# xbpeng/DeepMimic

Hardware: NVIDIA H100
Metric: env-steps/sec (30 Hz policy steps; humanoid3d_spinkick, 4096 envs/GPU) (higher is better)
Workload: dtype f32

## Files before the change

deepmimic_b200/csrc/kernels/dm_step.cu:

```cuda
#include "dm_model.cuh"
#include <type_traits>

namespace dmk {

namespace {

template <int W>
struct Tl {
    static __device__ __forceinline__ float shfl(float v, int src) { return __shfl_sync(0xffffffffu, v, src, W); }
    static __device__ __forceinline__ int shfli(int v, int src) { return __shfl_sync(0xffffffffu, v, src, W); }
    static __device__ __forceinline__ V3 shfl3(V3 v, int src) { return mk3(shfl(v.x, src), shfl(v.y, src), shfl(v.z, src)); }
    static __device__ __forceinline__ S6 shfl6(S6 v, int src) { return mks(shfl3(v.a, src), shfl3(v.l, src)); }
};
__device__ __forceinline__ void ld12(const float* p, float* o) {
    const float4 a = reinterpret_cast<const float4*>(p)[0], b = reinterpret_cast<const float4*>(p)[1], c_ = reinterpret_cast<const float4*>(p)[2];
    o[0] = a.x; o[1] = a.y; o[2] = a.z; o[3] = a.w; o[4] = b.x; o[5] = b.y; o[6] = b.z; o[7] = b.w; o[8] = c_.x; o[9] = c_.y; o[10] = c_.z; o[11] = c_.w;
}
__device__ __forceinline__ void st12(float* p, const float* o) {
    reinterpret_cast<float4*>(p)[0] = make_float4(o[0], o[1], o[2], o[3]); reinterpret_cast<float4*>(p)[1] = make_float4(o[4], o[5], o[6], o[7]);
    reinterpret_cast<float4*>(p)[2] = make_float4(o[8], o[9], o[10], o[11]);
}
__device__ __forceinline__ float rcp_fast(float x) { float r; asm("rcp.approx.ftz.f32 %0, %1;" : "=f"(r) : "f"(x)); return r; }
__device__ __forceinline__ int wmax(int v) {
#pragma unroll
    for (int o = 16; o > 0; o >>= 1) v = max(v, __shfl_xor_sync(0xffffffffu, v, o));
    return v;
}

struct Art {
    float ww[6];
    float wv[9];
    float vv[6];
};
__device__ __forceinline__ V3 wvT_mul(const float* g, V3 w) { return mk3(g[0] * w.x + g[3] * w.y + g[6] * w.z, g[1] * w.x + g[4] * w.y + g[7] * w.z, g[2] * w.x + g[5] * w.y + g[8] * w.z); }
__device__ __forceinline__ void rot_sym(const M3& R, const float* s, float* o) {
    float t[9];
#pragma unroll
    for (int j = 0; j < 3; ++j) {
        t[0 + j] = s[0] * R.m[j] + s[1] * R.m[3 + j] + s[2] * R.m[6 + j];
        t[3 + j] = s[1] * R.m[j] + s[3] * R.m[3 + j] + s[4] * R.m[6 + j];
        t[6 + j] = s[2] * R.m[j] + s[4] * R.m[3 + j] + s[5] * R.m[6 + j];
    }
    o[0] = R.m[0] * t[0] + R.m[3] * t[3] + R.m[6] * t[6];
    o[1] = R.m[0] * t[1] + R.m[3] * t[4] + R.m[6] * t[7];
    o[2] = R.m[0] * t[2] + R.m[3] * t[5] + R.m[6] * t[8];
    o[3] = R.m[1] * t[1] + R.m[4] * t[4] + R.m[7] * t[7];
    o[4] = R.m[1] * t[2] + R.m[4] * t[5] + R.m[7] * t[8];
    o[5] = R.m[2] * t[2] + R.m[5] * t[5] + R.m[8] * t[8];
}
__device__ __forceinline__ float normalize_angle3(float t) {
    float n = fmodf(t, 6.283185307179586f);
    if (n > 3.14159265358979f) n -= 6.283185307179586f;
    else if (n < -3.14159265358979f) n += 6.283185307179586f;
    return n;
}
__device__ __forceinline__ V3 quat_rotvec3(Q4 q) {
    float s = sqrtf(q.x * q.x + q.y * q.y + q.z * q.z);
    if (!(s > 0.000001f)) return mk3(0.f, 0.f, 0.f);
    float th = normalize_angle3(2.0f * atan2f(s, q.w));
    float k = th / s;
    return mk3(q.x * k, q.y * k, q.z * k);
}
__device__ __forceinline__ Q4 quat_integrate3(V3 omega, Q4 quat, bool base_body, float dt) {
    V3 angvel = base_body ? omega : qrot(quat, omega);
    float fAngle = sqrtf(dot(angvel, angvel));
    const float kThr = 0.5f * 1.57079632679489661923f;
    if (fAngle * dt > kThr) fAngle = kThr / dt;
    V3 axis;
    if (fAngle < 0.001f) axis = angvel * (0.5f * dt - (dt * dt * dt) * 0.020833333333f * fAngle * fAngle);
    else axis = angvel * (__sinf(0.5f * fAngle * dt) / fAngle);
    float cw = __cosf(fAngle * dt * 0.5f);
    Q4 r = base_body ? qmul(quat, mkq(-axis.x, -axis.y, -axis.z, cw)) : qmul(mkq(axis.x, axis.y, axis.z, cw), quat);
    float n = rsqrtf(r.x * r.x + r.y * r.y + r.z * r.z + r.w * r.w);
    return mkq(r.x * n, r.y * n, r.z * n, r.w * n);
}

enum LkSlot { kLC = 0 , kLM = 3,
              kLD = 4 , kLThr = 7,
              kLWd = 8 , kLInt = 14 , kLInt2 = 15 ,
              kLWb = 16 , kLFlg = 22 , kLTree = 23 ,
              kLAx = 24 , kLTl = 27,
              kLZr = 28 ,
              kLHe = 32 , kLKp = 35,
              kLKd = 36, kLLo = 37, kLHi = 38, kLChild = 39 ,
              kLDc = 40 , kLMc = 43 ,
              kLDyn = 44 , kLDChild = 45 ,
              kLkFloats = 48 };
__device__ __forceinline__ float4 ld4(const float* p) { return *reinterpret_cast<const float4*>(p); }
enum HdrSlot { kHLayout = 0, kHLvc = 24, kHGrav = 32 , kHh = 35, kHScale = 36, kHMu = 37, kHFdt = 38, kHDmax = 39 , kHdrFloats = 40 };
__device__ __forceinline__ float* step_smem() { extern __shared__ __align__(16) float dm_step_sm[]; return dm_step_sm; }

}

int dm_step_layout(int nl, int n, int chain_len, int maxrows, int W, StepLayout* L) {
    const int maxpts = maxrows / 3;
    int o = 0;
    L->nl = nl; L->n = n; L->chain_len = chain_len; L->maxrows = maxrows; L->maxpts = maxpts;
    L->oU = o; o += nl * 24;
    L->oR = o; o += nl * 12;
    L->oA = o;
    const int world = nl * 24, tri = maxrows * (maxrows + 1) / 2;
    L->oW = o; L->oV = o + nl * 12;
    L->oPp = o + world; L->oQ = L->oPp + maxpts * 4;
    const int pre = world + maxpts * 4 + 4 * 8;
    o += (pre > tri ? pre : tri);
    o = (o + 3) & ~3;
    const int ys = dm_step_y_stride(W), scr = 28 * (nl - 1);
    L->oY = o; o += (chain_len * ys > scr) ? chain_len * ys : scr;
    L->oLam = o; o += maxrows; o += (o & 1); L->oRhs = o; o += maxrows; L->oInv = o; o += maxrows;
    L->oRl = o; o += maxrows;
    L->oPi = o; o += maxpts; L->oPr = o; o += maxpts;
    L->oG = o; o += 21 + 13 + 2;
    L->oZ = o; o += ((n + 3) / 4) * 4;
    L->env_floats = ((o + 15) / 32) * 32 + 16;
    L->hot_floats = kHdrFloats + ((nl * kLkFloats + (nl * nl + nl * chain_len + 3) / 4 + 3) / 4) * 4;
    return L->hot_floats * 4 + 0;
}
int dm_step_smem_bytes(const StepLayout& L, int tiles) { return (L.hot_floats + L.env_floats * tiles) * static_cast<int>(sizeof(float)); }

constexpr int kSubstepBarriers = 2;
constexpr int kPgsBlock = 2;
enum PgsSection { kSecLimit = 0, kSecNormal = 1, kSecFriction = 2 };
// ... 808 lines not shown
            x[i] *= sG[15 + i];
        }
        dB = mks(mk3(x[0], x[1], x[2]), mk3(x[3], x[4], x[5]));
#pragma unroll
        for (int i = 0; i < 6; ++i) sB[7 + i] = cl100(sB[7 + i] + x[i]);
    }
    float z0 = 0.f, z1 = 0.f, z2 = 0.f, qd0 = 0.f, qd1 = 0.f, qd2 = 0.f;
    if (c.ndof >= 1) z0 = sZ[dof0] * u[21];
    if (c.ndof == 3) { z1 = sZ[dof0 + 1] * u[22]; z2 = sZ[dof0 + 2] * u[23]; }
    auto descend = [&](S6 a) {
        if (c.ndof >= 1) { qd0 = z0 - u[18] * (a.a.x * u[0] + a.a.y * u[1] + a.a.z * u[2] + a.l.x * u[3] + a.l.y * u[4] + a.l.z * u[5]); a.a += qd0 * S0; }
        if (c.ndof == 3) {
            qd1 = z1 - u[19] * (a.a.x * u[6] + a.a.y * u[7] + a.a.z * u[8] + a.l.x * u[9] + a.l.y * u[10] + a.l.z * u[11]); a.a += qd1 * S1;
            qd2 = z2 - u[20] * (a.a.x * u[12] + a.a.y * u[13] + a.a.z * u[14] + a.l.x * u[15] + a.l.y * u[16] + a.l.z * u[17]); a.a += qd2 * S2;
        }
        return a;
    };
    S6 al = mks(mk3(0, 0, 0), mk3(0, 0, 0));
    if (c.lane == 0) al = dB;
#pragma unroll 1
    for (int lv = 0; lv <= dmax; ++lv) {
        S6 pa = T::shfl6(al, dpar);
        if (dlev == lv) al = descend(shift_m(pa, cw));
    }
    __syncwarp();
    return make_float3(qd0, qd1, qd2);
}

template <int W>
__device__ __noinline__ void vel_pass(float jvx, float jvy, float jvz, bool want) {
    const Ctx c = make_ctx<W>();
    using T = Tl<W>;
    const StepLayout& LY = lay_of(c);
    const float* sS = c.E + LY.oR; float* sV = c.E + LY.oV; const float* sB = c.E + LY.oG + 21;
    float q[12];
    ld12(sS + c.li * 12, q);
    const V3 S0 = mk3(q[0], q[1], q[2]), S1 = mk3(q[3], q[4], q[5]), S2 = mk3(q[6], q[7], q[8]), cw = mk3(q[9], q[10], q[11]);
    V3 jww = mk3(0, 0, 0);
    if (c.jtype == kJSpherical) jww = jvx * S0 + jvy * S1 + jvz * S2; else if (c.jtype == kJRevolute) jww = jvx * S0;
    S6 vel = mks(mk3(0, 0, 0), mk3(0, 0, 0));
    if (c.lane == 0) { const V3 bo = mk3(sB[7], sB[8], sB[9]); vel = mks(bo + jww, mk3(sB[10], sB[11], sB[12]) + cross(bo, cw)); }
#pragma unroll 1
    for (int lv = 1; lv <= c.maxlevel; ++lv) {
        const S6 pv = T::shfl6(vel, c.plane);
        if (c.level == lv) vel = mks(pv.a + jww, pv.l + cross(pv.a, cw));
    }
    if (c.act && want) {
        float* v = sV + c.lane * 12;
        v[0] = vel.a.x; v[1] = vel.a.y; v[2] = vel.a.z; v[3] = vel.l.x; v[4] = vel.l.y; v[5] = vel.l.z;
    }
    __syncwarp();
}

template <int W, bool TASK>
__global__ void __launch_bounds__(kStepMaxThreads, 1) dm_step_kernel(const DevModel* __restrict__ gm, DevState st, const double* __restrict__ frame_times,
                                                                       const float* __restrict__ frames, double dt, int n_updates, int sim_substeps, StepLayout LY) {
    using T = Tl<W>;
    extern __shared__ __align__(16) float sm[];
    const int tiles = blockDim.x / W;
    const int tile = threadIdx.x / W;
    const int lane = threadIdx.x % W;
    const int slot = blockIdx.x * tiles + tile;
    const int env = (W == 16 && st.order) ? st.order[slot] : slot;
    const DevModel& M = *gm;
    const int nl = LY.nl, CL = LY.chain_len;
    const bool act = lane < nl;
    const int li = act ? lane : nl - 1;

    float* LK = sm + kHdrFloats;
    unsigned char* CD = reinterpret_cast<unsigned char*>(LK + nl * kLkFloats);
    unsigned char* CH = CD + nl * nl;
    int* LYS = reinterpret_cast<int*>(sm + kHLayout);
    for (int j = threadIdx.x; j < nl; j += blockDim.x) {
        const DevLink& K = M.link[j];
        float* q = LK + j * kLkFloats;
        const int p = K.parent;
        for (int k = 0; k < 3; ++k) { q[kLC + k] = K.evec[k] + (p >= 0 ? M.link[p].dvec[k] : 0.f); q[kLD + k] = K.dvec[k]; q[kLAx + k] = K.axis[k]; }
        q[kLM] = K.mass;
        auto lumped = [&](int c_) { const DevLink& C_ = M.link[c_]; return C_.ndof == 0 && C_.nchild == 0 && C_.parent >= 0 && M.link[C_.parent].ndof > 0; };
        const bool isroot = p < 0, self_lumped = lumped(j);
        {
            float cm = 0.f, mdx = 0.f, mdy = 0.f, mdz = 0.f, wD[6] = {0, 0, 0, 0, 0, 0}, wB[6] = {0, 0, 0, 0, 0, 0};
            auto add_part = [&](float m_, V3 r, const float* iD, const float* iB) {
                const float rr = dot(r, r);
                const float sh[6] = {m_ * (rr - r.x * r.x), -m_ * r.x * r.y, -m_ * r.x * r.z, m_ * (rr - r.y * r.y), -m_ * r.y * r.z, m_ * (rr - r.z * r.z)};
                for (int k = 0; k < 6; ++k) { wD[k] += iD[k] + sh[k]; wB[k] += iB[k] + sh[k]; }
                cm += m_; mdx += m_ * r.x; mdy += m_ * r.y; mdz += m_ * r.z;
            };
            if (!self_lumped) {
                V3 r = mk3(K.dvec[0], K.dvec[1], K.dvec[2]);
                if (isroot) r = r + mul(qmat(mkq(K.zrot[0], K.zrot[1], K.zrot[2], K.zrot[3])), mk3(K.evec[0], K.evec[1], K.evec[2]));
                const float iD[6] = {K.inertiaD[0], 0.f, 0.f, K.inertiaD[1], 0.f, K.inertiaD[2]}, iB[6] = {K.inertiaB[0], 0.f, 0.f, K.inertiaB[1], 0.f, K.inertiaB[2]};
                add_part(K.mass, r, iD, iB);
                for (int k = 0; k < K.nchild; ++k) {
                    const int c_ = K.child[k];
                    if (!lumped(c_)) continue;
                    const DevLink& C_ = M.link[c_];
                    const M3 Rc = qmat(mkq(C_.zrot[0], C_.zrot[1], C_.zrot[2], C_.zrot[3]));
                    const V3 rc = mk3(C_.evec[0] + K.dvec[0], C_.evec[1] + K.dvec[1], C_.evec[2] + K.dvec[2]) + mulT(Rc, mk3(C_.dvec[0], C_.dvec[1], C_.dvec[2]));
                    const float cD[6] = {C_.inertiaD[0], 0.f, 0.f, C_.inertiaD[1], 0.f, C_.inertiaD[2]}, cB[6] = {C_.inertiaB[0], 0.f, 0.f, C_.inertiaB[1], 0.f, C_.inertiaB[2]};
                    float rD[6], rB[6];
                    rot_sym(Rc, cD, rD); rot_sym(Rc, cB, rB);
                    add_part(C_.mass, rc, rD, rB);
                }
            }
            for (int k = 0; k < 6; ++k) { q[kLWd + k] = wD[k]; q[kLWb + k] = wB[k]; }
            q[kLMc] = cm;
            const float icm = cm > 0.f ? 1.0f / cm : 0.f;
            q[kLDc] = mdx * icm; q[kLDc + 1] = mdy * icm; q[kLDc + 2] = mdz * icm;
            int dch = 0, dn = 0;
            for (int k = 0; k < K.nchild; ++k) if (!lumped(K.child[k])) { dch |= (K.child[k] & 0xff) << (8 * dn); ++dn; }
            const int dlev = isroot ? -1 : (self_lumped ? 100 : K.level - 1);
            const int dpar = isroot ? 0 : p, byp = (!isroot && p >= 0 && M.link[p].parent < 0) ? p : 0xff;
            reinterpret_cast<int*>(q)[kLDyn] = (dpar & 0xff) | ((dlev & 0xff) << 8) | ((byp & 0xff) << 16) | ((dn & 0xff) << 24);
            reinterpret_cast<int*>(q)[kLDChild] = dch;
        }
        reinterpret_cast<int*>(q)[kLInt] = (K.parent & 0xff) | ((K.jtype & 0xff) << 8) | ((K.ndof & 0xff) << 16) | ((K.depth0 & 0xff) << 24);
        reinterpret_cast<int*>(q)[kLInt2] = (K.dof0 & 0xff) | ((K.last_depth & 0xff) << 8) | ((K.nchild & 0xff) << 16);
        for (int k = 0; k < 4; ++k) q[kLZr + k] = K.zrot[k];
        for (int k = 0; k < 3; ++k) q[kLHe + k] = K.he[k];
        q[kLThr] = K.break_thr; q[kLKp] = K.kp; q[kLKd] = K.kd; q[kLTl] = K.tlim; q[kLLo] = K.lim_lo; q[kLHi] = K.lim_hi;
        reinterpret_cast<int*>(q)[kLFlg] = (K.shape & 0xff) | ((K.fall_contact & 0xff) << 8) | ((K.has_limit & 0xff) << 16);
        reinterpret_cast<int*>(q)[kLTree] = (K.level & 0xff) | ((M.maxlevel & 0xff) << 8) | ((K.nchild & 0xff) << 16);
        reinterpret_cast<int*>(q)[kLChild] = (K.child[0] & 0xff) | ((K.child[1] & 0xff) << 8) | ((K.child[2] & 0xff) << 16) | ((K.child[3] & 0xff) << 24);
        for (int d = 0; d < CL; ++d) CH[j * CL + d] = M.chain_dof[j][d];
        for (int b = 0; b < nl; ++b) {
            int cnt = 0;
            const int lim = min(K.last_depth, M.link[b].last_depth);
            while (cnt <= lim && M.chain_dof[j][cnt] == M.chain_dof[b][cnt]) ++cnt;
            CD[j * nl + b] = static_cast<unsigned char>(cnt);
        }
    }
    if (threadIdx.x == blockDim.x - 1) {
        static_assert(sizeof(StepLayout) / sizeof(int) <= kHLvc, "StepLayout must fit the header slot");
        const int* src = reinterpret_cast<const int*>(&LY);
        for (int k = 0; k < static_cast<int>(sizeof(StepLayout) / sizeof(int)); ++k) LYS[k] = src[k];
        sm[kHGrav] = M.gravity[0]; sm[kHGrav + 1] = M.gravity[1]; sm[kHGrav + 2] = M.gravity[2];
        sm[kHh] = static_cast<float>(dt) / static_cast<float>(sim_substeps); sm[kHScale] = M.scale; sm[kHMu] = M.friction; sm[kHFdt] = static_cast<float>(dt);
    }
    if (threadIdx.x == 8) {
        int mx = 0;
        for (int j = 0; j < nl; ++j) { const DevLink& K = M.link[j]; if (K.parent >= 0 && !(K.ndof == 0 && K.nchild == 0 && M.link[K.parent].ndof > 0)) mx = max(mx, K.level - 1); }
        reinterpret_cast<int*>(sm)[kHDmax] = mx;
    }
    __syncthreads();

    float* E = sm + LY.hot_floats + tile * LY.env_floats;
    for (int k = lane * 4; k < LY.env_floats; k += W * 4) *reinterpret_cast<float4*>(E + k) = make_float4(0.f, 0.f, 0.f, 0.f);
    __syncwarp();
    float* sV = E + LY.oV; float* sG = E + LY.oG; float* sQ = E + LY.oQ; float* sLam = E + LY.oLam;
    const float* LKo = LK + li * kLkFloats;
    const int jtype = (reinterpret_cast<const int*>(LKo)[kLInt] >> 8) & 0xff, ndof = act ? ((reinterpret_cast<const int*>(LKo)[kLInt] >> 16) & 0xff) : 0;
    const int lflags = reinterpret_cast<const int*>(LKo)[kLFlg];
    const bool fall_contact = ((lflags >> 8) & 0xff) != 0, has_limit = ((lflags >> 16) & 0xff) != 0;

    const int ss = sim_stride(nl);
    float* sim = st.sim + static_cast<size_t>(env) * ss;
    double* tm = st.time + static_cast<size_t>(env) * kTimeDoubles;
    int* fl = st.flags + static_cast<size_t>(env) * kFlagInts;
    float* mani = st.manifold + static_cast<size_t>(env) * nl * kManifoldFloats;
    double* tk = nullptr;
    double* tkx = nullptr;
    if constexpr (TASK) { tk = st.task + static_cast<size_t>(env) * kTaskDoubles; tkx = st.taskx + static_cast<size_t>(env) * kTaskExtDoubles; }
    float* sB = sG + 21;
    if (lane == 0) {
        float4 b0 = reinterpret_cast<const float4*>(sim)[0], b1 = reinterpret_cast<const float4*>(sim)[1], b2 = reinterpret_cast<const float4*>(sim)[2],
               b3 = reinterpret_cast<const float4*>(sim)[3];
        sB[0] = b0.x; sB[1] = b0.y; sB[2] = b0.z; sB[3] = b1.x; sB[4] = b1.y; sB[5] = b1.z; sB[6] = b1.w;
        sB[7] = b2.x; sB[8] = b2.y; sB[9] = b2.z; sB[10] = b3.x; sB[11] = b3.y; sB[12] = b3.z;
    }
    float4 jp = reinterpret_cast<const float4*>(sim + 16)[li];
    float4 jv = reinterpret_cast<const float4*>(sim + 16 + 4 * nl)[li];
    int need_action = fl[kFNeedAction];
    int cbits = 0;
    bool alive = fl[kFDone] == 0;
    int f_over = fl[kFRowOverflow], f_updates = fl[kFUpdates];
    __syncwarp();

    const float h = static_cast<float>(dt) / static_cast<float>(sim_substeps);
    const float fdt = static_cast<float>(dt);
    const float gx = M.gravity[0], gy = M.gravity[1], gz = M.gravity[2];
    const float scale = M.scale, mu = M.friction;

    float tau0 = 0.f, tau1 = 0.f, tau2 = 0.f;
    bool in_contact_tol = false;

#ifdef DM_PROFILE
    unsigned int* PRF = reinterpret_cast<unsigned int*>(sm + LY.hot_floats + tiles * LY.env_floats) + (threadIdx.x / 32) * kProfCounters;
    if ((threadIdx.x & 31) == 0) for (int k = 0; k < kProfCounters; ++k) PRF[k] = 0u;
    unsigned int prf_t = static_cast<unsigned int>(clock64());
#define PROF(sec) do { if ((threadIdx.x & 31) == 0) { unsigned int t_ = static_cast<unsigned int>(clock64()); PRF[sec] += t_ - prf_t; prf_t = t_; } } while (0)
    unsigned int* PRFP = PRF;
#else
#define PROF(sec) do { } while (0)
    unsigned int* PRFP = nullptr;
#endif
    bool need_kin = true, pending_flags = false;
    int mcnt = 4;
    int last_nr = 0;
    const int stages_per_upd = sim_substeps + 1;
    const int total_stages = n_updates * stages_per_upd;
#pragma unroll 1
    for (int stage = 0; stage <= total_stages; ++stage) {
        if ((stage % stages_per_upd) != 0 && act && alive && mcnt > 0) {
            const float* mp_ = mani + li * kManifoldFloats;
            asm volatile("prefetch.global.L1 [%0];" ::"l"(mp_));
            asm volatile("prefetch.global.L1 [%0];" ::"l"(mp_ + 32));
        }
        if (need_kin) { need_kin = false; kin_pass<W>(jp, jv); }
        PROF(0);
        if (pending_flags) {
            pending_flags = false;
            need_action = cbits & 1;
            const unsigned fb = __ballot_sync(0xffffffffu, act && fall_contact && in_contact_tol);
            const unsigned fseg = (W == 32) ? fb : ((fb >> (threadIdx.x & 16)) & 0xffffu);
            const int fallen = (fseg != 0 && M.enable_contact_fall) ? 1 : 0;
            const float* v = sV + li * 12;
            const V3 wa = mk3(v[0], v[1], v[2]);
            const V3 vw = (mk3(v[3], v[4], v[5]) + cross(wa, mk3(v[6], v[7], v[8]))) * (1.0f / scale);
            float mx = fmaxf(fmaxf(fmaxf(fabsf(vw.x), fabsf(vw.y)), fabsf(vw.z)), fmaxf(fmaxf(fabsf(wa.x), fabsf(wa.y)), fabsf(wa.z)));
            const unsigned eb = __ballot_sync(0xffffffffu, act && mx > 100.f);
            const unsigned eseg = (W == 32) ? eb : ((eb >> (threadIdx.x & 16)) & 0xffffu);
            int task_fail = 0;
            int fallen_eff = fallen;
            if constexpr (TASK) {
                const V3 com = tile_com<W>(E + LY.oW + li * 12, v, act ? LKo[kLM] : 0.f, 1.0f / (M.total_mass * scale));
                const int kind = M.task_kind;
                TaskBodies B;
                if (kind >= kTaskHeadingGetup) {
                    const float* w_ = E + LY.oW + li * 12;
                    const V3 cpos = mk3((w_[9] + v[6]) / scale, (w_[10] + v[7]) / scale, (w_[11] + v[8]) / scale);
                    const TaskExtParams& X = M.taskx;
                    B.head_y = T::shfl(cpos.y, X.head_id);
                    B.contact_fall = fallen;
#pragma unroll
                    for (int k = 0; k < kMaxTaskBodies; ++k) {
                        const V3 sp = T::shfl3(cpos, k < X.n_strike ? X.strike_bodies[k] : 0), sv = T::shfl3(vw, k < X.n_strike ? X.strike_bodies[k] : 0);
                        const V3 fp = T::shfl3(cpos, k < X.n_fail ? X.fail_bodies[k] : 0);
                        B.spos[k][0] = sp.x; B.spos[k][1] = sp.y; B.spos[k][2] = sp.z; B.svel[k][0] = sv.x; B.svel[k][1] = sv.y; B.svel[k][2] = sv.z;
                        B.fpos[k][0] = fp.x; B.fpos[k][1] = fp.y; B.fpos[k][2] = fp.z;
                    }
                }
                int tf = 0, fe = fallen;
                if (lane == 0 && alive) {
                    TaskRng rng{M.task_seed, M.env_id_base + static_cast<unsigned long long>(env), tk + kKCounter};
                    const double rx = static_cast<double>(sB[0]) / M.scale, rz = static_cast<double>(sB[2]) / M.scale;
                    tk[kKCom] = com.x; tk[kKCom + 1] = com.y; tk[kKCom + 2] = com.z;
                    if (kind == kTaskStrike) {
                        const double scene_time = tm[kTTimer];
                        tk[kKTimer] += dt;
                        strike_update(M.taskx, tk, tkx, rx, rz, scene_time, B);
                        if (tk[kKTimer] >= tk[kKTimerMax]) task_timer_reset(M.task, tk, rng);
                        tf = strike_terminate(M.task, M.taskx, tk, tkx, rx, rz, scene_time);
                    } else {
                        task_update(task_base_kind(kind), M.task, tk, rng, dt, rx, rz);
                        tf = task_dist_fail(kind, M.task, tk, rx, rz) ? 1 : 0;
                        if (kind == kTaskHeadingGetup) {
                            tkx[kXHeadY] = B.head_y;
                            if (getup_update(M.taskx, tkx, dt, M.test_mode != 0, fallen != 0)) fe = 0;
                        }
                    }
                }
                task_fail = T::shfli(tf, 0);
                fallen_eff = T::shfli(fe, 0);
            }
            if (alive) {
                int term = (M.enable_fall_end && fallen_eff) ? 1 : 0;
                if (!term && (cbits & 4)) term = 1;
                if (TASK && !term && task_fail) term = task_fail;
                f_updates++;
                const bool end = (cbits & 2) || term;
                if (end || stage == total_stages) {
                    if (lane == 0) {
                        reinterpret_cast<float4*>(sim)[0] = make_float4(sB[0], sB[1], sB[2], 0.f);
                        reinterpret_cast<float4*>(sim)[1] = make_float4(sB[3], sB[4], sB[5], sB[6]);
                        reinterpret_cast<float4*>(sim)[2] = make_float4(sB[7], sB[8], sB[9], 0.f);
                        reinterpret_cast<float4*>(sim)[3] = make_float4(sB[10], sB[11], sB[12], 0.f);
                        fl[kFNeedAction] = need_action; fl[kFDone] = end ? 1 : 0; fl[kFTerminate] = term; fl[kFValid] = (eseg == 0) ? 1 : 0; fl[kFFallen] = fallen_eff;
                        fl[kFRowOverflow] = f_over; fl[kFUpdates] = f_updates;
                        if (W == 16) st.load[env] = last_nr;
                    }
                    if (act) {
                        reinterpret_cast<float4*>(sim + 16)[lane] = jp;
                        reinterpret_cast<float4*>(sim + 16 + 4 * nl)[lane] = jv;
                    }
                }
                if (end) alive = false;
            }
        }
        PROF(1);
        if (stage == total_stages) break;
        if (__syncthreads_and(!alive)) break;
        PROF(2);
        if (__ballot_sync(0xffffffffu, alive) == 0u) {
            if ((stage % stages_per_upd) != 0)
                for (int k = 0; k < kSubstepBarriers; ++k) __syncthreads();
            continue;
        }
        const int ph = stage % stages_per_upd;
        if (ph == 0) {
            int cb = 0;
            if constexpr (TASK) {
                if (__ballot_sync(0xffffffffu, alive && need_action) != 0u) {
                    const V3 com = tile_com<W>(E + LY.oW + li * 12, sV + li * 12, act ? LKo[kLM] : 0.f, 1.0f / (M.total_mass * scale));
                    if (lane == 0 && alive && need_action) { tk[kKPrevCom] = com.x; tk[kKPrevCom + 1] = com.y; tk[kKPrevCom + 2] = com.z; }
                }
            }
            if (lane == 0 && alive) {
                const double timer = tm[kTTimer] + dt;
                double kin_time = tm[kTKin];
                double dur_ = M.motion_dur;
                if constexpr (TASK) dur_ = st.ctab->info[st.clip[env]].dur;
                const double dur = dur_;
                double p0 = kin_time / dur; p0 -= floor(p0);
                kin_time += dt;
                double p1 = kin_time / dur; p1 -= floor(p1);
                if constexpr (TASK) {
                    const ClipInfo& ci = st.ctab->info[st.clip[env]];
                    if (ci.loop && p1 < p0 && M.sync_root_pos) {
                        const double simq[4] = {static_cast<double>(sB[3]), static_cast<double>(sB[4]), static_cast<double>(sB[5]), static_cast<double>(sB[6])};
                        kin_wrap_sync(frame_times + ci.frame_off, frames + static_cast<size_t>(ci.frame_off) * M.pose_dim, M.pose_dim, ci.num_frames, ci.cycle_delta, dur, kin_time,
                                      tm + kTOrigin, tm + kTOriginRot, static_cast<double>(sB[0]) / M.scale, static_cast<double>(sB[2]) / M.scale, simq, true, false);
                    }
                } else if (M.loop_motion && p1 < p0 && (M.sync_root_pos || M.sync_root_rot)) {
                    const double simq[4] = {static_cast<double>(sB[3]), static_cast<double>(sB[4]), static_cast<double>(sB[5]), static_cast<double>(sB[6])};
                    kin_wrap_sync(frame_times, frames, M.pose_dim, M.num_frames, M.cycle_delta, dur, kin_time, tm + kTOrigin, tm + kTOriginRot,
                                  static_cast<double>(sB[0]) / M.scale, static_cast<double>(sB[2]) / M.scale, simq, M.sync_root_pos != 0, M.sync_root_rot != 0);
                }
                const double ctrl_time = tm[kTCtrl] + dt;
                if (need_action) tm[kTPrevAct] = ctrl_time;
                tm[kTTimer] = timer; tm[kTKin] = kin_time; tm[kTCtrl] = ctrl_time;
                {
                    const double cur = ctrl_time + tm[kTInitOff], pad = 0.001 * dt, T_ = M.query_dt;
                    int c0 = static_cast<int>(floor((cur + pad) / T_)), c1 = static_cast<int>(floor((cur + pad - dt) / T_));
                    cb = (c0 != c1) ? 1 : 0;
                }
                if (timer >= tm[kTTimerMax]) cb |= 2;
                if (M.end_at_clip_end && kin_time >= dur) cb |= 4;
            }
            cbits = T::shfli(cb, 0);
            need_action = 0;
            PROF(3);
            const float4 tg = reinterpret_cast<const float4*>(sim + 16 + 8 * nl)[li];
            float e0 = 0, e1 = 0, e2 = 0;
            if (jtype == kJSpherical) {
                Q4 q = mkq(jp.x, jp.y, jp.z, jp.w);
                Q4 dq = qmul(q, mkq(jv.x, jv.y, jv.z, 0.f));
                Q4 qi = qnormalize(mkq(q.x + 0.5f * fdt * dq.x, q.y + 0.5f * fdt * dq.y, q.z + 0.5f * fdt * dq.z, q.w + 0.5f * fdt * dq.w));
                V3 e = quat_rotvec3(qmul(qconj(qi), mkq(tg.x, tg.y, tg.z, tg.w)));
                e0 = e.x; e1 = e.y; e2 = e.z;
            } else if (jtype == kJRevolute) {
                e0 = tg.x - (normalize_angle3(jp.x) + fdt * jv.x);
            }
            const float kp = LKo[kLKp], kd = LKo[kLKd];
            const float pe0 = kp * e0, pe1 = kp * e1, pe2 = kp * e2;
            const float3 qdd = aba_solve<W>(pe0 - kd * jv.x, pe1 - kd * jv.y, pe2 - kd * jv.z, fdt * kd, 0, jv.x, jv.y, jv.z);
            float t0 = 0, t1 = 0, t2 = 0;
            if (ndof >= 1) t0 = pe0 + kd * (-jv.x - fdt * qdd.x);
            if (ndof == 3) { t1 = pe1 + kd * (-jv.y - fdt * qdd.y); t2 = pe2 + kd * (-jv.z - fdt * qdd.z); }
            const float mag = sqrtf(t0 * t0 + t1 * t1 + t2 * t2), tlim = LKo[kLTl];
            if (mag > tlim) { float s = tlim / mag; t0 *= s; t1 *= s; t2 *= s; }
            tau0 = t0; tau1 = t1; tau2 = t2;
            PROF(4);
            continue;
        }
        int P;
        {
            const int r = collide<W>(mani, alive ? 1 : 0, mcnt);
            P = r & 0xff; in_contact_tol = ((r >> 8) & 1) != 0; if ((r >> 9) & 1) f_over = 1; mcnt = (r >> 10) & 7;
        }
        PROF(3);
        {
            const float3 qdd = aba_solve<W>(tau0, tau1, tau2, 0.f, 1, jv.x, jv.y, jv.z);
            bool hit = false;
            if (ndof >= 1) { const float v = jv.x + h * qdd.x; jv.x = cl100(v); hit |= fabsf(v) > 100.f; }
            if (ndof == 3) { const float v1 = jv.y + h * qdd.y, v2 = jv.z + h * qdd.z; jv.y = cl100(v1); jv.z = cl100(v2); hit |= fabsf(v1) > 100.f || fabsf(v2) > 100.f; }
            if (lane == 0) for (int k = 0; k < 6; ++k) hit |= fabsf(sB[7 + k]) >= 100.f;
            const unsigned hb = __ballot_sync(0xffffffffu, hit);
            if (hb != 0u) {
                const unsigned hseg = (W == 32) ? hb : ((hb >> (threadIdx.x & 16)) & 0xffffu);
                vel_pass<W>(jv.x, jv.y, jv.z, hseg != 0u);
            }
        }
        PROF(ph == 1 ? 16 : 17);
        __syncthreads();
        PROF(2);
        int lim_dir = 0; float lim_pen = 0.f;
        if (act && has_limit && alive) {
            float p0 = jp.x - LKo[kLLo], p1 = LKo[kLHi] - jp.x;
            if (!(p0 > 0.f)) { lim_dir = 1; lim_pen = p0; }
            else if (!(p1 > 0.f)) { lim_dir = -1; lim_pen = p1; }
        }
        const unsigned lbal = __ballot_sync(0xffffffffu, lim_dir != 0);
        const unsigned lseg = (W == 32) ? lbal : ((lbal >> (threadIdx.x & 16)) & 0xffffu);
        int NL = __popc(lseg);
        const unsigned anyrow = __ballot_sync(0xffffffffu, NL + P > 0);
        last_nr = 0;
        if (anyrow != 0) {
            {
                const int lidx = __popc(lseg & ((1u << lane) - 1u));
                if (NL > 8) { NL = 8; f_over = 1; }
                if (lim_dir != 0 && lidx < 8) { sQ[lidx] = __int_as_float(lane); sQ[8 + lidx] = (lim_dir == -1) ? -1.f : 1.f; sQ[16 + lidx] = lim_pen; sQ[24 + lidx] = jv.x; }
            }
            if (NL + 3 * P > LY.maxrows) { P = (LY.maxrows - NL) / 3; f_over = 1; }
            const int NR = NL + 3 * P;
            last_nr = NR;
            __syncwarp();
            PROF(5);
#ifdef DM_PROFILE
            { const int nrm = wmax(NR); if ((threadIdx.x & 31) == 0) { PRF[13] += nrm; PRF[14] += 1; if (nrm > W) PRF[15] += 1; } }
#endif
            solve_rows<W>(NL, P, mani, alive ? 1 : 0, PRFP);
            PROF(10);
            const float3 dq = dv_pass<W>();
            if (NR > 0) {
                if (ndof >= 1) jv.x = cl100(jv.x + dq.x);
                if (ndof == 3) { jv.y = cl100(jv.y + dq.y); jv.z = cl100(jv.z + dq.z); }
            }
            PROF(11);
        }
        __syncthreads();
        PROF(2);
        if (lane == 0) {
            sB[0] += h * sB[10]; sB[1] += h * sB[11]; sB[2] += h * sB[12];
            const Q4 q = quat_integrate3(mk3(sB[7], sB[8], sB[9]), mkq(sB[3], sB[4], sB[5], sB[6]), true, h);
            sB[3] = q.x; sB[4] = q.y; sB[5] = q.z; sB[6] = q.w;
        }
        if (jtype == kJRevolute) jp.x += h * jv.x;
        else if (jtype == kJSpherical) { Q4 q = quat_integrate3(mk3(jv.x, jv.y, jv.z), mkq(jp.x, jp.y, jp.z, jp.w), false, h); jp = make_float4(q.x, q.y, q.z, q.w); }
        __syncwarp();
        need_kin = true;
        if (ph == sim_substeps) pending_flags = true;
        PROF(12);
    }
#ifdef DM_PROFILE
    __syncwarp();
    if ((threadIdx.x & 31) == 0 && st.prof) { unsigned int* o = st.prof + (blockIdx.x * (blockDim.x / 32) + threadIdx.x / 32) * kProfCounters; for (int k = 0; k < kProfCounters; ++k) o[k] = PRF[k]; }
#endif
}

const StepKernel kStepKernels[2][2] = {{dm_step_kernel<16, false>, dm_step_kernel<16, true>}, {dm_step_kernel<32, false>, dm_step_kernel<32, true>}};

constexpr int kEnvOrderItems = 4;
__global__ void __launch_bounds__(kEnvOrderThreads) dm_env_order_kernel(const int* __restrict__ load, int n_padded, int tiles, int W, int* __restrict__ order) {
    constexpr int kWarps = kEnvOrderThreads / 32, kCells = kEnvOrderItems * kWarps, kChunk = kEnvOrderItems * kEnvOrderThreads;
    constexpr int kParts = kEnvOrderThreads / kLoadBuckets, kPer = kCells / kParts;
    static_assert(kParts <= 32 && 32 % kParts == 0 && kCells % kParts == 0, "the scan of a bucket's cells runs inside one warp");
    __shared__ int base[kLoadBuckets];
    __shared__ int cnt[kLoadBuckets][kCells + 1];
    const int t = threadIdx.x, warp = t / 32, lane = t % 32;
    const unsigned lt = (1u << lane) - 1u;
    int b[kEnvOrderItems];
    auto load_chunk = [&](int c0) {
#pragma unroll
        for (int i = 0; i < kEnvOrderItems; ++i) { const int e = c0 + i * kEnvOrderThreads + t; b[i] = (e < n_padded) ? env_load_bucket(load[e]) : kLoadBuckets; }
    };
    auto count = [&](int bk) {
        const unsigned peers = __match_any_sync(0xffffffffu, bk);
        if (bk < kLoadBuckets && (peers & lt) == 0) atomicAdd(&base[bk], __popc(peers));
    };
    load_chunk(0);
    if (t < kLoadBuckets) base[t] = 0;
    __syncthreads();
#pragma unroll
    for (int i = 0; i < kEnvOrderItems; ++i) count(b[i]);
    for (int e = kChunk + t; e < n_padded + t; e += kEnvOrderThreads) count((e < n_padded) ? env_load_bucket(load[e]) : kLoadBuckets);
    __syncthreads();
    if (warp == 0) {
        const int c0 = base[2 * lane], c1 = base[2 * lane + 1];
        int incl = c0 + c1;
#pragma unroll
        for (int o = 1; o < 32; o <<= 1) { const int v = __shfl_up_sync(0xffffffffu, incl, o); if (lane >= o) incl += v; }
        base[2 * lane] = incl - c0 - c1; base[2 * lane + 1] = incl - c1;
    }
    const int sb = t / kParts, part = t % kParts;
    for (int c0 = 0; c0 < n_padded; c0 += kChunk) {
        if (c0 > 0) load_chunk(c0);
        for (int k = t; k < kLoadBuckets * (kCells + 1); k += kEnvOrderThreads) (&cnt[0][0])[k] = 0;
        __syncthreads();
        int below[kEnvOrderItems];
#pragma unroll
        for (int i = 0; i < kEnvOrderItems; ++i) {
            const unsigned peers = __match_any_sync(0xffffffffu, b[i]);
            below[i] = __popc(peers & lt);
            if (b[i] < kLoadBuckets && below[i] == 0) cnt[b[i]][i * kWarps + warp] = __popc(peers);
// ... 26 lines not shown
```

Baseline: 2.528 million.

## Pack step-loop state into a bitfield and rematerialize per-env pointers

The kernel's long-lived loop state (alive, need_kin, pending flags, clock bits, manifold count, contact points, row count, overflow) moves into one packed 32-bit word. Per-env pointers and per-link constants are recomputed on demand from tid, shared memory and global state rather than held across the whole loop, and the update counter moves into shared memory. The aim is to reduce register pressure in the single-block-per-SM step kernel and avoid spills. The cost is extra bit manipulation and address arithmetic each time a value is used. A small FMA rewrite in the quaternion integrator is included.

```diff
diff --git a/deepmimic_b200/csrc/kernels/dm_step.cu b/deepmimic_b200/csrc/kernels/dm_step.cu
--- a/deepmimic_b200/csrc/kernels/dm_step.cu
+++ b/deepmimic_b200/csrc/kernels/dm_step.cu
@@ -67,7 +67,7 @@
     const float kThr = 0.5f * 1.57079632679489661923f;
     if (fAngle * dt > kThr) fAngle = kThr / dt;
     V3 axis;
-    if (fAngle < 0.001f) axis = angvel * (0.5f * dt - (dt * dt * dt) * 0.020833333333f * fAngle * fAngle);
+    if (fAngle < 0.001f) axis = angvel * __fmaf_rn(-fAngle, (dt * dt * dt) * 0.020833333333f * fAngle, 0.5f * dt);
     else axis = angvel * (__sinf(0.5f * fAngle * dt) / fAngle);
     float cw = __cosf(fAngle * dt * 0.5f);
     Q4 r = base_body ? qmul(quat, mkq(-axis.x, -axis.y, -axis.z, cw)) : qmul(mkq(axis.x, axis.y, axis.z, cw), quat);
@@ -982,6 +982,48 @@
     __syncwarp();
 }
 
+enum LoopField : int {
+    kLsAlive = 0 + 32, kLsNeedKin = 1 + 32, kLsPendingFlags = 2 + 32, kLsNeedAction = 3 + 32,
+    kLsContactTol = 4 + 32,
+    kLsOver = 5 + 32,
+    kLsClock = 6 + 3 * 32,
+    kLsMcnt = 9 + 3 * 32,
+    kLsNpts = 12 + 5 * 32,
+    kLsRows = 17 + 8 * 32
+};
+static_assert(dm_step_y_stride(32) / 3 < 32 && dm_step_y_stride(32) < 256, "contact points and solver rows must fit their LoopBits fields");
+struct LoopBits {
+    unsigned w = 0;
+    __device__ __forceinline__ unsigned get(LoopField f) const { return (w >> (f & 31)) & ((1u << (f >> 5)) - 1u); }
+    __device__ __forceinline__ void set(LoopField f, unsigned v) { const unsigned m = ((1u << (f >> 5)) - 1u) << (f & 31); w = (w & ~m) | ((v << (f & 31)) & m); }
+};
+constexpr int kBUpdates = 13;
+template <int W>
+struct EnvRefs {
+    int tid, lane, li, env;
+    bool act;
+    float* E;
+    float* sB;
+    const float* LKo;
+    float* sim; double* tm; int* fl; float* mani;
+    __device__ __forceinline__ EnvRefs(const DevState& st, const StepLayout& LY, int env_id) {
+        asm volatile("mov.u32 %0, %%tid.x;" : "=r"(tid));
+        env = env_id;
+        asm volatile("" : "+r"(env));
+        lane = tid % W;
+        act = lane < LY.nl;
+        li = act ? lane : LY.nl - 1;
+        E = step_smem() + LY.hot_floats + (tid / W) * LY.env_floats;
+        sB = E + LY.oG + 21;
+        LKo = step_smem() + kHdrFloats + li * kLkFloats;
+        sim = st.sim + static_cast<size_t>(env) * sim_stride(LY.nl);
+        tm = st.time + static_cast<size_t>(env) * kTimeDoubles;
+        fl = st.flags + static_cast<size_t>(env) * kFlagInts;
+        mani = st.manifold + static_cast<size_t>(env) * LY.nl * kManifoldFloats;
+    }
+    __device__ __forceinline__ int lk_int(int slot) const { return reinterpret_cast<const int*>(LKo)[slot]; }
+};
+
 template <int W, bool TASK>
 __global__ void __launch_bounds__(kStepMaxThreads, 1) dm_step_kernel(const DevModel* __restrict__ gm, DevState st, const double* __restrict__ frame_times,
                                                                        const float* __restrict__ frames, double dt, int n_updates, int sim_substeps, StepLayout LY) {
@@ -1075,45 +1117,32 @@
     }
     __syncthreads();
 
-    float* E = sm + LY.hot_floats + tile * LY.env_floats;
-    for (int k = lane * 4; k < LY.env_floats; k += W * 4) *reinterpret_cast<float4*>(E + k) = make_float4(0.f, 0.f, 0.f, 0.f);
-    __syncwarp();
-    float* sV = E + LY.oV; float* sG = E + LY.oG; float* sQ = E + LY.oQ; float* sLam = E + LY.oLam;
-    const float* LKo = LK + li * kLkFloats;
-    const int jtype = (reinterpret_cast<const int*>(LKo)[kLInt] >> 8) & 0xff, ndof = act ? ((reinterpret_cast<const int*>(LKo)[kLInt] >> 16) & 0xff) : 0;
-    const int lflags = reinterpret_cast<const int*>(LKo)[kLFlg];
-    const bool fall_contact = ((lflags >> 8) & 0xff) != 0, has_limit = ((lflags >> 16) & 0xff) != 0;
-
-    const int ss = sim_stride(nl);
-    float* sim = st.sim + static_cast<size_t>(env) * ss;
-    double* tm = st.time + static_cast<size_t>(env) * kTimeDoubles;
-    int* fl = st.flags + static_cast<size_t>(env) * kFlagInts;
-    float* mani = st.manifold + static_cast<size_t>(env) * nl * kManifoldFloats;
-    double* tk = nullptr;
-    double* tkx = nullptr;
-    if constexpr (TASK) { tk = st.task + static_cast<size_t>(env) * kTaskDoubles; tkx = st.taskx + static_cast<size_t>(env) * kTaskExtDoubles; }
-    float* sB = sG + 21;
-    if (lane == 0) {
-        float4 b0 = reinterpret_cast<const float4*>(sim)[0], b1 = reinterpret_cast<const float4*>(sim)[1], b2 = reinterpret_cast<const float4*>(sim)[2],
-               b3 = reinterpret_cast<const float4*>(sim)[3];
-        sB[0] = b0.x; sB[1] = b0.y; sB[2] = b0.z; sB[3] = b1.x; sB[4] = b1.y; sB[5] = b1.z; sB[6] = b1.w;
-        sB[7] = b2.x; sB[8] = b2.y; sB[9] = b2.z; sB[10] = b3.x; sB[11] = b3.y; sB[12] = b3.z;
-    }
-    float4 jp = reinterpret_cast<const float4*>(sim + 16)[li];
-    float4 jv = reinterpret_cast<const float4*>(sim + 16 + 4 * nl)[li];
-    int need_action = fl[kFNeedAction];
-    int cbits = 0;
-    bool alive = fl[kFDone] == 0;
-    int f_over = fl[kFRowOverflow], f_updates = fl[kFUpdates];
-    __syncwarp();
-
-    const float h = static_cast<float>(dt) / static_cast<float>(sim_substeps);
-    const float fdt = static_cast<float>(dt);
-    const float gx = M.gravity[0], gy = M.gravity[1], gz = M.gravity[2];
-    const float scale = M.scale, mu = M.friction;
+    float4 jp, jv;
+    LoopBits ls;
+    {
+        const EnvRefs<W> r(st, LY, env);
+        for (int k = lane * 4; k < LY.env_floats; k += W * 4) *reinterpret_cast<float4*>(r.E + k) = make_float4(0.f, 0.f, 0.f, 0.f);
+        __syncwarp();
+        float* sB = r.sB;
+        const float* sim = r.sim;
+        if (lane == 0) {
+            float4 b0 = reinterpret_cast<const float4*>(sim)[0], b1 = reinterpret_cast<const float4*>(sim)[1], b2 = reinterpret_cast<const float4*>(sim)[2],
+                   b3 = reinterpret_cast<const float4*>(sim)[3];
+            sB[0] = b0.x; sB[1] = b0.y; sB[2] = b0.z; sB[3] = b1.x; sB[4] = b1.y; sB[5] = b1.z; sB[6] = b1.w;
+            sB[7] = b2.x; sB[8] = b2.y; sB[9] = b2.z; sB[10] = b3.x; sB[11] = b3.y; sB[12] = b3.z;
+            reinterpret_cast<int*>(sB)[kBUpdates] = r.fl[kFUpdates];
+        }
+        jp = reinterpret_cast<const float4*>(sim + 16)[li];
+        jv = reinterpret_cast<const float4*>(sim + 16 + 4 * nl)[li];
+        ls.set(kLsNeedAction, r.fl[kFNeedAction] != 0);
+        ls.set(kLsAlive, r.fl[kFDone] == 0);
+        ls.set(kLsOver, r.fl[kFRowOverflow] != 0);
+        ls.set(kLsNeedKin, 1);
+        ls.set(kLsMcnt, 4);
+        __syncwarp();
+    }
 
     float tau0 = 0.f, tau1 = 0.f, tau2 = 0.f;
-    bool in_contact_tol = false;
 
 #ifdef DM_PROFILE
     unsigned int* PRF = reinterpret_cast<unsigned int*>(sm + LY.hot_floats + tiles * LY.env_floats) + (threadIdx.x / 32) * kProfCounters;
@@ -1125,32 +1154,38 @@
 #define PROF(sec) do { } while (0)
     unsigned int* PRFP = nullptr;
 #endif
-    bool need_kin = true, pending_flags = false;
-    int mcnt = 4;
-    int last_nr = 0;
     const int stages_per_upd = sim_substeps + 1;
     const int total_stages = n_updates * stages_per_upd;
 #pragma unroll 1
     for (int stage = 0; stage <= total_stages; ++stage) {
-        if ((stage % stages_per_upd) != 0 && act && alive && mcnt > 0) {
-            const float* mp_ = mani + li * kManifoldFloats;
-            asm volatile("prefetch.global.L1 [%0];" ::"l"(mp_));
-            asm volatile("prefetch.global.L1 [%0];" ::"l"(mp_ + 32));
-        }
-        if (need_kin) { need_kin = false; kin_pass<W>(jp, jv); }
+        if ((stage % stages_per_upd) != 0 && ls.get(kLsAlive) && ls.get(kLsMcnt) > 0) {
+            const EnvRefs<W> r(st, LY, env);
+            if (r.act) {
+                const float* mp_ = r.mani + r.li * kManifoldFloats;
+                asm volatile("prefetch.global.L1 [%0];" ::"l"(mp_));
+                asm volatile("prefetch.global.L1 [%0];" ::"l"(mp_ + 32));
+            }
+        }
+        if (ls.get(kLsNeedKin)) { ls.set(kLsNeedKin, 0); kin_pass<W>(jp, jv); }
         PROF(0);
-        if (pending_flags) {
-            pending_flags = false;
-            need_action = cbits & 1;
-            const unsigned fb = __ballot_sync(0xffffffffu, act && fall_contact && in_contact_tol);
-            const unsigned fseg = (W == 32) ? fb : ((fb >> (threadIdx.x & 16)) & 0xffffu);
+        if (ls.get(kLsPendingFlags)) {
+            ls.set(kLsPendingFlags, 0);
+            ls.set(kLsNeedAction, ls.get(kLsClock) & 1);
+            const EnvRefs<W> r(st, LY, env);
+            const int lane = r.lane, li = r.li;
+            const bool act = r.act;
+            float* E = r.E; float* sB = r.sB; const float* LKo = r.LKo;
+            const float scale = step_smem()[kHScale];
+            const bool fall_contact = ((r.lk_int(kLFlg) >> 8) & 0xff) != 0;
+            const unsigned fb = __ballot_sync(0xffffffffu, act && fall_contact && ls.get(kLsContactTol));
+            const unsigned fseg = (W == 32) ? fb : ((fb >> (r.tid & 16)) & 0xffffu);
             const int fallen = (fseg != 0 && M.enable_contact_fall) ? 1 : 0;
-            const float* v = sV + li * 12;
+            const float* v = E + LY.oV + li * 12;
             const V3 wa = mk3(v[0], v[1], v[2]);
             const V3 vw = (mk3(v[3], v[4], v[5]) + cross(wa, mk3(v[6], v[7], v[8]))) * (1.0f / scale);
             float mx = fmaxf(fmaxf(fmaxf(fabsf(vw.x), fabsf(vw.y)), fabsf(vw.z)), fmaxf(fmaxf(fabsf(wa.x), fabsf(wa.y)), fabsf(wa.z)));
             const unsigned eb = __ballot_sync(0xffffffffu, act && mx > 100.f);
-            const unsigned eseg = (W == 32) ? eb : ((eb >> (threadIdx.x & 16)) & 0xffffu);
+            const unsigned eseg = (W == 32) ? eb : ((eb >> (r.tid & 16)) & 0xffffu);
             int task_fail = 0;
             int fallen_eff = fallen;
             if constexpr (TASK) {
@@ -1172,8 +1207,11 @@
                     }
                 }
                 int tf = 0, fe = fallen;
-                if (lane == 0 && alive) {
-                    TaskRng rng{M.task_seed, M.env_id_base + static_cast<unsigned long long>(env), tk + kKCounter};
+                if (lane == 0 && ls.get(kLsAlive)) {
+                    double* tk = st.task + static_cast<size_t>(r.env) * kTaskDoubles;
+                    double* tkx = st.taskx + static_cast<size_t>(r.env) * kTaskExtDoubles;
+                    const double* tm = r.tm;
+                    TaskRng rng{M.task_seed, M.env_id_base + static_cast<unsigned long long>(r.env), tk + kKCounter};
                     const double rx = static_cast<double>(sB[0]) / M.scale, rz = static_cast<double>(sB[2]) / M.scale;
                     tk[kKCom] = com.x; tk[kKCom + 1] = com.y; tk[kKCom + 2] = com.z;
                     if (kind == kTaskStrike) {
@@ -1194,59 +1232,66 @@
                 task_fail = T::shfli(tf, 0);
                 fallen_eff = T::shfli(fe, 0);
             }
-            if (alive) {
+            if (ls.get(kLsAlive)) {
                 int term = (M.enable_fall_end && fallen_eff) ? 1 : 0;
-                if (!term && (cbits & 4)) term = 1;
+                if (!term && (ls.get(kLsClock) & 4)) term = 1;
                 if (TASK && !term && task_fail) term = task_fail;
-                f_updates++;
-                const bool end = (cbits & 2) || term;
+                if (lane == 0) ++reinterpret_cast<int*>(sB)[kBUpdates];
+                const bool end = (ls.get(kLsClock) & 2) || term;
                 if (end || stage == total_stages) {
+                    float* sim = r.sim; int* fl = r.fl;
                     if (lane == 0) {
                         reinterpret_cast<float4*>(sim)[0] = make_float4(sB[0], sB[1], sB[2], 0.f);
                         reinterpret_cast<float4*>(sim)[1] = make_float4(sB[3], sB[4], sB[5], sB[6]);
                         reinterpret_cast<float4*>(sim)[2] = make_float4(sB[7], sB[8], sB[9], 0.f);
                         reinterpret_cast<float4*>(sim)[3] = make_float4(sB[10], sB[11], sB[12], 0.f);
-                        fl[kFNeedAction] = need_action; fl[kFDone] = end ? 1 : 0; fl[kFTerminate] = term; fl[kFValid] = (eseg == 0) ? 1 : 0; fl[kFFallen] = fallen_eff;
-                        fl[kFRowOverflow] = f_over; fl[kFUpdates] = f_updates;
-                        if (W == 16) st.load[env] = last_nr;
+                        fl[kFNeedAction] = ls.get(kLsNeedAction); fl[kFDone] = end ? 1 : 0; fl[kFTerminate] = term; fl[kFValid] = (eseg == 0) ? 1 : 0; fl[kFFallen] = fallen_eff;
+                        fl[kFRowOverflow] = ls.get(kLsOver); fl[kFUpdates] = reinterpret_cast<const int*>(sB)[kBUpdates];
+                        if (W == 16) st.load[r.env] = ls.get(kLsRows);
                     }
                     if (act) {
                         reinterpret_cast<float4*>(sim + 16)[lane] = jp;
                         reinterpret_cast<float4*>(sim + 16 + 4 * nl)[lane] = jv;
                     }
                 }
-                if (end) alive = false;
+                if (end) ls.set(kLsAlive, 0);
             }
         }
         PROF(1);
         if (stage == total_stages) break;
-        if (__syncthreads_and(!alive)) break;
+        if (__syncthreads_and(!ls.get(kLsAlive))) break;
         PROF(2);
-        if (__ballot_sync(0xffffffffu, alive) == 0u) {
+        if (__ballot_sync(0xffffffffu, ls.get(kLsAlive)) == 0u) {
             if ((stage % stages_per_upd) != 0)
                 for (int k = 0; k < kSubstepBarriers; ++k) __syncthreads();
             continue;
         }
         const int ph = stage % stages_per_upd;
         if (ph == 0) {
+            const EnvRefs<W> r(st, LY, env);
+            const int lane = r.lane, li = r.li;
+            float* sB = r.sB;
             int cb = 0;
             if constexpr (TASK) {
-                if (__ballot_sync(0xffffffffu, alive && need_action) != 0u) {
-                    const V3 com = tile_com<W>(E + LY.oW + li * 12, sV + li * 12, act ? LKo[kLM] : 0.f, 1.0f / (M.total_mass * scale));
-                    if (lane == 0 && alive && need_action) { tk[kKPrevCom] = com.x; tk[kKPrevCom + 1] = com.y; tk[kKPrevCom + 2] = com.z; }
+                if (__ballot_sync(0xffffffffu, ls.get(kLsAlive) && ls.get(kLsNeedAction)) != 0u) {
+                    const float scale = step_smem()[kHScale];
+                    const V3 com = tile_com<W>(r.E + LY.oW + li * 12, r.E + LY.oV + li * 12, r.act ? r.LKo[kLM] : 0.f, 1.0f / (M.total_mass * scale));
+                    double* tk = st.task + static_cast<size_t>(r.env) * kTaskDoubles;
+                    if (lane == 0 && ls.get(kLsAlive) && ls.get(kLsNeedAction)) { tk[kKPrevCom] = com.x; tk[kKPrevCom + 1] = com.y; tk[kKPrevCom + 2] = com.z; }
                 }
             }
-            if (lane == 0 && alive) {
+            if (lane == 0 && ls.get(kLsAlive)) {
+                double* tm = r.tm;
                 const double timer = tm[kTTimer] + dt;
                 double kin_time = tm[kTKin];
                 double dur_ = M.motion_dur;
-                if constexpr (TASK) dur_ = st.ctab->info[st.clip[env]].dur;
+                if constexpr (TASK) dur_ = st.ctab->info[st.clip[r.env]].dur;
                 const double dur = dur_;
                 double p0 = kin_time / dur; p0 -= floor(p0);
                 kin_time += dt;
                 double p1 = kin_time / dur; p1 -= floor(p1);
                 if constexpr (TASK) {
-                    const ClipInfo& ci = st.ctab->info[st.clip[env]];
+                    const ClipInfo& ci = st.ctab->info[st.clip[r.env]];
                     if (ci.loop && p1 < p0 && M.sync_root_pos) {
                         const double simq[4] = {static_cast<double>(sB[3]), static_cast<double>(sB[4]), static_cast<double>(sB[5]), static_cast<double>(sB[6])};
                         kin_wrap_sync(frame_times + ci.frame_off, frames + static_cast<size_t>(ci.frame_off) * M.pose_dim, M.pose_dim, ci.num_frames, ci.cycle_delta, dur, kin_time,
@@ -1258,7 +1303,7 @@
                                   static_cast<double>(sB[0]) / M.scale, static_cast<double>(sB[2]) / M.scale, simq, M.sync_root_pos != 0, M.sync_root_rot != 0);
                 }
                 const double ctrl_time = tm[kTCtrl] + dt;
-                if (need_action) tm[kTPrevAct] = ctrl_time;
+                if (ls.get(kLsNeedAction)) tm[kTPrevAct] = ctrl_time;
                 tm[kTTimer] = timer; tm[kTKin] = kin_time; tm[kTCtrl] = ctrl_time;
                 {
                     const double cur = ctrl_time + tm[kTInitOff], pad = 0.001 * dt, T_ = M.query_dt;
@@ -1268,47 +1313,59 @@
                 if (timer >= tm[kTTimerMax]) cb |= 2;
                 if (M.end_at_clip_end && kin_time >= dur) cb |= 4;
             }
-            cbits = T::shfli(cb, 0);
-            need_action = 0;
+            ls.set(kLsClock, T::shfli(cb, 0));
+            ls.set(kLsNeedAction, 0);
             PROF(3);
-            const float4 tg = reinterpret_cast<const float4*>(sim + 16 + 8 * nl)[li];
-            float e0 = 0, e1 = 0, e2 = 0;
-            if (jtype == kJSpherical) {
-                Q4 q = mkq(jp.x, jp.y, jp.z, jp.w);
-                Q4 dq = qmul(q, mkq(jv.x, jv.y, jv.z, 0.f));
-                Q4 qi = qnormalize(mkq(q.x + 0.5f * fdt * dq.x, q.y + 0.5f * fdt * dq.y, q.z + 0.5f * fdt * dq.z, q.w + 0.5f * fdt * dq.w));
-                V3 e = quat_rotvec3(qmul(qconj(qi), mkq(tg.x, tg.y, tg.z, tg.w)));
-                e0 = e.x; e1 = e.y; e2 = e.z;
-            } else if (jtype == kJRevolute) {
-                e0 = tg.x - (normalize_angle3(jp.x) + fdt * jv.x);
-            }
-            const float kp = LKo[kLKp], kd = LKo[kLKd];
-            const float pe0 = kp * e0, pe1 = kp * e1, pe2 = kp * e2;
-            const float3 qdd = aba_solve<W>(pe0 - kd * jv.x, pe1 - kd * jv.y, pe2 - kd * jv.z, fdt * kd, 0, jv.x, jv.y, jv.z);
+            float pe0, pe1, pe2;
+            float3 qdd;
+            {
+                const float fdt = step_smem()[kHFdt];
+                const int jtype = (r.lk_int(kLInt) >> 8) & 0xff;
+                const float4 tg = reinterpret_cast<const float4*>(r.sim + 16 + 8 * nl)[li];
+                float e0 = 0, e1 = 0, e2 = 0;
+                if (jtype == kJSpherical) {
+                    Q4 q = mkq(jp.x, jp.y, jp.z, jp.w);
+                    Q4 dq = qmul(q, mkq(jv.x, jv.y, jv.z, 0.f));
+                    Q4 qi = qnormalize(mkq(q.x + 0.5f * fdt * dq.x, q.y + 0.5f * fdt * dq.y, q.z + 0.5f * fdt * dq.z, q.w + 0.5f * fdt * dq.w));
+                    V3 e = quat_rotvec3(qmul(qconj(qi), mkq(tg.x, tg.y, tg.z, tg.w)));
+                    e0 = e.x; e1 = e.y; e2 = e.z;
+                } else if (jtype == kJRevolute) {
+                    e0 = tg.x - (normalize_angle3(jp.x) + fdt * jv.x);
+                }
+                const float kp = r.LKo[kLKp], kd = r.LKo[kLKd];
+                pe0 = kp * e0; pe1 = kp * e1; pe2 = kp * e2;
+                qdd = aba_solve<W>(pe0 - kd * jv.x, pe1 - kd * jv.y, pe2 - kd * jv.z, fdt * kd, 0, jv.x, jv.y, jv.z);
+            }
+            const EnvRefs<W> r2(st, LY, env);
+            const float fdt = step_smem()[kHFdt], kd = r2.LKo[kLKd];
+            const int ndof = r2.act ? ((r2.lk_int(kLInt) >> 16) & 0xff) : 0;
             float t0 = 0, t1 = 0, t2 = 0;
             if (ndof >= 1) t0 = pe0 + kd * (-jv.x - fdt * qdd.x);
             if (ndof == 3) { t1 = pe1 + kd * (-jv.y - fdt * qdd.y); t2 = pe2 + kd * (-jv.z - fdt * qdd.z); }
-            const float mag = sqrtf(t0 * t0 + t1 * t1 + t2 * t2), tlim = LKo[kLTl];
+            const float mag = sqrtf(t0 * t0 + t1 * t1 + t2 * t2), tlim = r2.LKo[kLTl];
             if (mag > tlim) { float s = tlim / mag; t0 *= s; t1 *= s; t2 *= s; }
             tau0 = t0; tau1 = t1; tau2 = t2;
             PROF(4);
             continue;
         }
-        int P;
+        if (ph == sim_substeps) ls.set(kLsPendingFlags, 1);
         {
-            const int r = collide<W>(mani, alive ? 1 : 0, mcnt);
-            P = r & 0xff; in_contact_tol = ((r >> 8) & 1) != 0; if ((r >> 9) & 1) f_over = 1; mcnt = (r >> 10) & 7;
+            const int r = collide<W>(EnvRefs<W>(st, LY, env).mani, ls.get(kLsAlive) ? 1 : 0, ls.get(kLsMcnt));
+            ls.set(kLsNpts, r & 0xff); ls.set(kLsContactTol, (r >> 8) & 1); if ((r >> 9) & 1) ls.set(kLsOver, 1); ls.set(kLsMcnt, (r >> 10) & 7);
         }
         PROF(3);
         {
             const float3 qdd = aba_solve<W>(tau0, tau1, tau2, 0.f, 1, jv.x, jv.y, jv.z);
+            const EnvRefs<W> r(st, LY, env);
+            const float h = step_smem()[kHh];
+            const int ndof = r.act ? ((r.lk_int(kLInt) >> 16) & 0xff) : 0;
             bool hit = false;
             if (ndof >= 1) { const float v = jv.x + h * qdd.x; jv.x = cl100(v); hit |= fabsf(v) > 100.f; }
             if (ndof == 3) { const float v1 = jv.y + h * qdd.y, v2 = jv.z + h * qdd.z; jv.y = cl100(v1); jv.z = cl100(v2); hit |= fabsf(v1) > 100.f || fabsf(v2) > 100.f; }
-            if (lane == 0) for (int k = 0; k < 6; ++k) hit |= fabsf(sB[7 + k]) >= 100.f;
+            if (r.lane == 0) for (int k = 0; k < 6; ++k) hit |= fabsf(r.sB[7 + k]) >= 100.f;
             const unsigned hb = __ballot_sync(0xffffffffu, hit);
             if (hb != 0u) {
-                const unsigned hseg = (W == 32) ? hb : ((hb >> (threadIdx.x & 16)) & 0xffffu);
+                const unsigned hseg = (W == 32) ? hb : ((hb >> (r.tid & 16)) & 0xffffu);
                 vel_pass<W>(jv.x, jv.y, jv.z, hseg != 0u);
             }
         }
@@ -1316,34 +1373,40 @@
         __syncthreads();
         PROF(2);
         int lim_dir = 0; float lim_pen = 0.f;
-        if (act && has_limit && alive) {
-            float p0 = jp.x - LKo[kLLo], p1 = LKo[kLHi] - jp.x;
+        const EnvRefs<W> r(st, LY, env);
+        const bool has_limit = ((r.lk_int(kLFlg) >> 16) & 0xff) != 0;
+        if (r.act && has_limit && ls.get(kLsAlive)) {
+            float p0 = jp.x - r.LKo[kLLo], p1 = r.LKo[kLHi] - jp.x;
             if (!(p0 > 0.f)) { lim_dir = 1; lim_pen = p0; }
             else if (!(p1 > 0.f)) { lim_dir = -1; lim_pen = p1; }
         }
         const unsigned lbal = __ballot_sync(0xffffffffu, lim_dir != 0);
-        const unsigned lseg = (W == 32) ? lbal : ((lbal >> (threadIdx.x & 16)) & 0xffffu);
+        const unsigned lseg = (W == 32) ? lbal : ((lbal >> (r.tid & 16)) & 0xffffu);
         int NL = __popc(lseg);
+        int P = ls.get(kLsNpts);
         const unsigned anyrow = __ballot_sync(0xffffffffu, NL + P > 0);
-        last_nr = 0;
+        ls.set(kLsRows, 0);
         if (anyrow != 0) {
             {
-                const int lidx = __popc(lseg & ((1u << lane) - 1u));
-                if (NL > 8) { NL = 8; f_over = 1; }
-                if (lim_dir != 0 && lidx < 8) { sQ[lidx] = __int_as_float(lane); sQ[8 + lidx] = (lim_dir == -1) ? -1.f : 1.f; sQ[16 + lidx] = lim_pen; sQ[24 + lidx] = jv.x; }
-            }
-            if (NL + 3 * P > LY.maxrows) { P = (LY.maxrows - NL) / 3; f_over = 1; }
+                const int lidx = __popc(lseg & ((1u << r.lane) - 1u));
+                if (NL > 8) { NL = 8; ls.set(kLsOver, 1); }
+                float* sQ = r.E + LY.oQ;
+                if (lim_dir != 0 && lidx < 8) { sQ[lidx] = __int_as_float(r.lane); sQ[8 + lidx] = (lim_dir == -1) ? -1.f : 1.f; sQ[16 + lidx] = lim_pen; sQ[24 + lidx] = jv.x; }
+            }
+            if (NL + 3 * P > LY.maxrows) { P = (LY.maxrows - NL) / 3; ls.set(kLsOver, 1); }
             const int NR = NL + 3 * P;
-            last_nr = NR;
+            ls.set(kLsRows, NR);
             __syncwarp();
             PROF(5);
 #ifdef DM_PROFILE
             { const int nrm = wmax(NR); if ((threadIdx.x & 31) == 0) { PRF[13] += nrm; PRF[14] += 1; if (nrm > W) PRF[15] += 1; } }
 #endif
-            solve_rows<W>(NL, P, mani, alive ? 1 : 0, PRFP);
+            solve_rows<W>(NL, P, r.mani, ls.get(kLsAlive) ? 1 : 0, PRFP);
             PROF(10);
             const float3 dq = dv_pass<W>();
-            if (NR > 0) {
+            if (ls.get(kLsRows) > 0) {
+                const EnvRefs<W> r2(st, LY, env);
+                const int ndof = r2.act ? ((r2.lk_int(kLInt) >> 16) & 0xff) : 0;
                 if (ndof >= 1) jv.x = cl100(jv.x + dq.x);
                 if (ndof == 3) { jv.y = cl100(jv.y + dq.y); jv.z = cl100(jv.z + dq.z); }
             }
@@ -1351,7 +1414,11 @@
         }
         __syncthreads();
         PROF(2);
-        if (lane == 0) {
+        const EnvRefs<W> r3(st, LY, env);
+        const float h = step_smem()[kHh];
+        const int jtype = (r3.lk_int(kLInt) >> 8) & 0xff;
+        if (r3.lane == 0) {
+            float* sB = r3.sB;
             sB[0] += h * sB[10]; sB[1] += h * sB[11]; sB[2] += h * sB[12];
             const Q4 q = quat_integrate3(mk3(sB[7], sB[8], sB[9]), mkq(sB[3], sB[4], sB[5], sB[6]), true, h);
             sB[3] = q.x; sB[4] = q.y; sB[5] = q.z; sB[6] = q.w;
@@ -1359,8 +1426,7 @@
         if (jtype == kJRevolute) jp.x += h * jv.x;
         else if (jtype == kJSpherical) { Q4 q = quat_integrate3(mk3(jv.x, jv.y, jv.z), mkq(jp.x, jp.y, jp.z, jp.w), false, h); jp = make_float4(q.x, q.y, q.z, q.w); }
         __syncwarp();
-        need_kin = true;
-        if (ph == sim_substeps) pending_flags = true;
+        ls.set(kLsNeedKin, 1);
         PROF(12);
     }
 #ifdef DM_PROFILE
```

Result: faster. 2.774 million (median of 6 runs) (+9.7%).
